# QData/ChromeGCN

Measured on AMD Instinct MI355X. Metric: GCN windows/sec (2-layer, d_model=128) on GM12878 Hi-C graph, higher is better.
Workload: dtype f32

## Files before the change

### chromegcn_amd/csrc/cgcn_head.hip

```cpp
#include "cgcn_common.hpp"

#define HEAD_STAT_BLOCKS 128
#define HEAD_TILE 16
#define HEADB_TILE 32
#ifndef HEAD_MAX_PARTIALS
#define HEAD_MAX_PARTIALS 256
#endif


template <int D>
__global__ __launch_bounds__(256) void k_head_colstats(int n, int S, int rows_per_blk, const float* __restrict__ X,
                                                       float* __restrict__ part) {
  constexpr int RL = 256 / D;
  __shared__ float sm[2][256];
  const int c = threadIdx.x % D, rl = threadIdx.x / D;
  const int r0 = blockIdx.x * rows_per_blk, r1 = min(n, r0 + rows_per_blk);
  for (int s = 0; s < S; ++s) {
    const float* Xs = X + (size_t)s * n * D + c;
    const float pivot = r0 < n ? fmaxf(Xs[(size_t)r0 * D], 0.f) : 0.f;
    float s1 = 0.f, s2 = 0.f;
    int i = r0 + rl;
    for (; i + 3 * RL < r1; i += 4 * RL) {
      float v[4];
#pragma unroll
// ... 1130 lines not shown
#pragma unroll
      for (int t = 0; t < RPW; ++t) {
        const int i = node0 + own + t * 8;
#pragma unroll
        for (int s = 0; s < 2; ++s) {
          if (i < n && s < S) ld_row<EPL>(xv[t][s], &X[(unsigned)((s * n + i) * D + lane * EPL)]);
          else zero_row<EPL>(xv[t][s]);
        }
      }
    };
    auto load_targets = [&](int tile) {
      const int node0 = tile * TR;
      const int j = own * 16 + (lane & 15), q = lane >> 4;
#pragma unroll
      for (int mb = 0; mb < NRB; ++mb)
#pragma unroll
        for (int e = 0; e < 4; ++e) {
          const int i = node0 + mb * 16 + q * 4 + e;
          tgv[mb][e] = (i < n && j < Cp) ? target[(unsigned)(i * C + c0 + j)] : 0.f;
        }
    };
    if (mt > 0) {
      load_rows(blockIdx.x);
      load_targets(blockIdx.x);
    }
    __syncthreads();
#pragma unroll
    for (int e = 0; e < EPL; ++e)
#pragma unroll
      for (int s = 0; s < 2; ++s) head_stat<D>(sa, stash, mean, invstd, s < S ? s : 0, lane * EPL + e, mu[s][e], is[s][e]);
    for (int k = 0; k <= mt; ++k) {
      const int tile = (int)blockIdx.x + k * G;
      const int node0 = tile * TR;
      RS_STAMP(0);
      if (k < mt) {
        int lane_ = lane;
        asm volatile("" : "+v"(lane_));
        float* __restrict__ Yb = Yt[k & 1];
#pragma unroll
        for (int t = 0; t < RPW; ++t) {
          const int rr = own + t * 8;
          const int i = node0 + rr;
          f32x2 ym;
#pragma unroll
          for (int e = 0; e < EPL; ++e) {
            float y[2];
#pragma unroll
            for (int s = 0; s < 2; ++s) {
              y[s] = (fmaxf(xv[t][s][e], 0.f) - mu[s][e]) * is[s][e] * gw[e] + gb[e];
              if (DROP) y[s] = dropout_keep(key, (uint32_t)((s * n + i) * D + lane_ * EPL + e), thresh) ? y[s] * keep_scale : 0.f;
            }
            const float a = y[0] + (S2 ? y[1] : 0.f);
            ym[e] = i < n ? a * invS : 0.f;
          }
          *(f32x2*)&Yb[rr * LDY + lane_ * EPL] = ym;
        }
      }
      RS_STAMP(1);
      __syncthreads();
      RS_STAMP(2);
      f32x4 acc[NRB];
#pragma unroll
      for (int mb = 0; mb < NRB; ++mb) acc[mb] = (f32x4){0.f, 0.f, 0.f, 0.f};
      if (k < mt) {
        if (k + 1 < mt) load_rows(tile + G);
        if (own < NB) {
          OPAQUE_LANE(r, q, lq);
          __builtin_amdgcn_s_setprio(HEAD_RS_PRIO);
          const float* __restrict__ Ya = Yt[k & 1] + r * LDY + 4 * q;
          const float* __restrict__ Wa = Wl + (own * 16 + r) * LDW + 4 * q;
#pragma unroll
          for (int t = 0; t < KQ / 4; ++t) {
            f32x4 a[NRB];
#pragma unroll
            for (int mb = 0; mb < NRB; ++mb) a[mb] = *(const f32x4*)&Ya[mb * 16 * LDY + 16 * t];
            const f32x4 b = *(const f32x4*)&Wa[16 * t];
#pragma unroll
            for (int u = 0; u < 4; ++u)
#pragma unroll
              for (int mb = 0; mb < NRB; ++mb) acc[mb] = __builtin_amdgcn_mfma_f32_16x16x4f32(a[mb][u], b[u], acc[mb], 0, 0, 0);
          }
          __builtin_amdgcn_s_setprio(0);
        }
      }
      RS_STAMP(3);
      __syncthreads();
      RS_STAMP(4);
      if (k < mt) {
        float* __restrict__ Pb = Pt[k & 1];
        OPAQUE_LANE(r, q, lq);
        const int j = own * 16 + r;
#pragma unroll
        for (int mb = 0; mb < NRB; ++mb)
#pragma unroll
          for (int e = 0; e < 4; ++e) {
            const int row = mb * 16 + q * 4 + e;
            const int i = node0 + row;
            const bool ok = i < n && j < Cp;
            const float pred = acc[mb][e] + bj;
            const float en = __expf(-fabsf(pred));
            const float inv = __builtin_amdgcn_rcpf(1.f + en);
            const float p = pred >= 0.f ? inv : en * inv;
            const float l = fmaxf(pred, 0.f) - pred * tgv[mb][e] + __logf(1.f + en);
            lacc += ok ? l : 0.f;
            if (ok) {
              if (HEAD_NT_PROBS) __builtin_nontemporal_store(p, &probs[(unsigned)(i * C + c0 + j)]);
              else probs[(unsigned)(i * C + c0 + j)] = p;
            }
            const float dp = ok ? (p - tgv[mb][e]) * inv_count : 0.f;
            dbo += dp;
            Pb[row * LDP + j] = dp;
          }
        if (k + 1 < mt) load_targets(tile + G);
      }
      RS_STAMP(5);
      __syncthreads();
    }
    dbo += __shfl_xor(dbo, 16);
    dbo += __shfl_xor(dbo, 32);
    if ((lane >> 4) == 0 && c0 + own * 16 + (lane & 15) < CPT) P[CPT * D + c0 + own * 16 + (lane & 15)] = dbo;
    lacc = wave_sum(lacc);
    if (lane == 0) lsum[own] = lacc;
    __syncthreads();
    if (threadIdx.x == 0) {
      float t = 0.f;
#pragma unroll
      for (int w = 0; w < 8; ++w) t += lsum[w];
      const float tl = first ? t : loss_part[blockIdx.x] + t;
      loss_part[blockIdx.x] = tl;
#ifndef HRSX_NOTICKET
      if (sa.acc && last) head_loss_ticket(sa, S, D, tl, inv_count);
#endif
    }
  } else {
    f32x4 accW[NB];
#pragma unroll
    for (int i = 0; i < NB; ++i) accW[i] = (f32x4){0.f, 0.f, 0.f, 0.f};
    float sdy[2] = {0.f, 0.f}, sdyx[2] = {0.f, 0.f}, mu[2], is[2];
    __syncthreads();
    if (sa.acc && blockIdx.x == 0 && first && wave == 8) head_stat_bookkeeping<D>(sa, stash, S, lane);
#pragma unroll
    for (int s = 0; s < 2; ++s) head_stat<D>(sa, stash, mean, invstd, s < S ? s : 0, own * 16 + (lane & 15), mu[s], is[s]);
    float xq[2][NRB][4];
    auto load_xq = [&](int tile) {
      OPAQUE_LANE(r, q, lq);
      const int node0 = tile * TR, c = own * 16 + r;
#pragma unroll
      for (int s = 0; s < 2; ++s)
#pragma unroll
        for (int mb = 0; mb < NRB; ++mb)
#pragma unroll
          for (int e = 0; e < 4; ++e) {
            const int i = node0 + mb * 16 + q * 4 + e;
            xq[s][mb][e] = (last && i < n && s < S) ? X[(unsigned)((s * n + i) * D + c)] : 0.f;
          }
    };
    for (int k = 0; k <= mt; ++k) {
      const int node0 = ((int)blockIdx.x + (k - 1) * G) * TR;
      f32x4 accY[NRB];
#pragma unroll
      for (int mb = 0; mb < NRB; ++mb) accY[mb] = (f32x4){0.f, 0.f, 0.f, 0.f};
      RS_STAMP(0);
      if (k >= 1) {
        const float* __restrict__ Pb = Pt[(k - 1) & 1];
        OPAQUE_LANE(r, q, lq);
        if (MULTI && !first) {
          const int c = own * 16 + r;
#pragma unroll
          for (int mb = 0; mb < NRB; ++mb)
#pragma unroll
            for (int e = 0; e < 4; ++e) {
              const int i = node0 + mb * 16 + q * 4 + e;
              accY[mb][e] = i < n ? dym[(unsigned)(i * D + c)] : 0.f;
            }
        }
        __builtin_amdgcn_s_setprio(HEAD_RS_PRIO);
        const float* __restrict__ Pa = Pb + r * LDP + q;
        const float* __restrict__ Wa = Wl + q * LDW + own * 16 + r;
        float pa[2][4 * NRB], wb[2][4];
#pragma unroll
        for (int u = 0; u < 4; ++u) {
          wb[0][u] = Wa[4 * u * LDW];
#pragma unroll
          for (int mb = 0; mb < NRB; ++mb) pa[0][u * NRB + mb] = Pa[mb * 16 * LDP + 4 * u];
        }
#pragma unroll
        for (int g = 0; g < NB; ++g) {
          if (g + 1 < NB) {
#pragma unroll
            for (int u = 0; u < 4; ++u) {
              wb[(g + 1) & 1][u] = Wa[4 * (4 * (g + 1) + u) * LDW];
#pragma unroll
              for (int mb = 0; mb < NRB; ++mb) pa[(g + 1) & 1][u * NRB + mb] = Pa[mb * 16 * LDP + 4 * (4 * (g + 1) + u)];
            }
          }
          __builtin_amdgcn_sched_barrier(0);
#pragma unroll
          for (int u = 0; u < 4; ++u)
#pragma unroll
            for (int mb = 0; mb < NRB; ++mb) accY[mb] = __builtin_amdgcn_mfma_f32_16x16x4f32(pa[g & 1][u * NRB + mb], wb[g & 1][u], accY[mb], 0, 0, 0);
          __builtin_amdgcn_sched_barrier(0);
        }
        __builtin_amdgcn_s_setprio(0);
      }
      RS_STAMP(1);
      __syncthreads();
      RS_STAMP(2);
      if (k >= 1) {
        OPAQUE_LANE(r, q, lq);
        const int c = own * 16 + r;
#pragma unroll
        for (int mb = 0; mb < NRB; ++mb)
#pragma unroll
          for (int e = 0; e < 4; ++e) {
            const int i = node0 + mb * 16 + q * 4 + e;
            const float g = accY[mb][e];
            if (i < n) dym[(unsigned)(i * D + c)] = g;
            if (last) {
#pragma unroll
              for (int s = 0; s < 2; ++s) {
                float dy = g * invS;
                if (DROP) dy = dropout_keep(key, (uint32_t)((s * n + i) * D + c), thresh) ? dy * keep_scale : 0.f;
                if (s == 1) dy = S2 ? dy : 0.f;
                const float xh = (fmaxf(xq[s][mb][e], 0.f) - mu[s]) * is[s];
                sdy[s] += dy;
                sdyx[s] += dy * xh;
              }
            }
          }
      }
      RS_STAMP(3);
      __syncthreads();
      RS_STAMP(4);
      if (k < mt) load_xq((int)blockIdx.x + k * G);
      if (k >= 1) {
        OPAQUE_LANE(r, q, lq);
        __builtin_amdgcn_s_setprio(HEAD_RS_PRIO);
        const float* __restrict__ Pa = Pt[(k - 1) & 1] + q * LDP + r;
        const float* __restrict__ Ya = Yt[(k - 1) & 1] + q * LDY + own * 16 + r;
        float a0[NB], a1[NB], b0, b1;
        b0 = Ya[0];
#pragma unroll
        for (int ib = 0; ib < NB; ++ib) a0[ib] = Pa[ib * 16];
#pragma unroll
        for (int kk = 0; kk < TR / 4; kk += 2) {
          b1 = Ya[(kk + 1) * 4 * LDY];
#pragma unroll
          for (int ib = 0; ib < NB; ++ib) a1[ib] = Pa[(kk + 1) * 4 * LDP + ib * 16];
          __builtin_amdgcn_sched_barrier(0);
#pragma unroll
          for (int ib = 0; ib < NB; ++ib) accW[ib] = __builtin_amdgcn_mfma_f32_16x16x4f32(a0[ib], b0, accW[ib], 0, 0, 0);
          __builtin_amdgcn_sched_barrier(0);
          if (kk + 2 < TR / 4) {
            b0 = Ya[(kk + 2) * 4 * LDY];
#pragma unroll
            for (int ib = 0; ib < NB; ++ib) a0[ib] = Pa[(kk + 2) * 4 * LDP + ib * 16];
          }
          __builtin_amdgcn_sched_barrier(0);
#pragma unroll
          for (int ib = 0; ib < NB; ++ib) accW[ib] = __builtin_amdgcn_mfma_f32_16x16x4f32(a1[ib], b1, accW[ib], 0, 0, 0);
          __builtin_amdgcn_sched_barrier(0);
        }
        __builtin_amdgcn_s_setprio(0);
      }
      RS_STAMP(5);
      __syncthreads();
    }
    const int r = lane & 15, q = lane >> 4;
#pragma unroll
    for (int ib = 0; ib < CBMAX; ++ib)
#pragma unroll
      for (int e = 0; e < 4; ++e) {
        const float v = ib < NB ? accW[ib < NB ? ib : 0][e] : 0.f;
        if (c0 + ib * 16 < CPT) P[(size_t)(c0 + ib * 16 + q * 4 + e) * D + own * 16 + r] = v;
      }
    if (last) {
      double* out = (double*)(P + CPT * D + CPT);
#pragma unroll
      for (int s = 0; s < 2; ++s) {
        double a = (double)sdy[s], b = (double)sdyx[s];
        a += __shfl_xor(a, 16); a += __shfl_xor(a, 32);
        b += __shfl_xor(b, 16); b += __shfl_xor(b, 32);
        if (q == 0) {
          out[s * D + own * 16 + r] = a;
          out[(2 + s) * D + own * 16 + r] = b;
          if (sa.acc && s < S) {
            int fa, fb;
            head_bacc_points(wmax, 16, keep_scale, n, fa, fb);
            unsigned long long* bb = bacc_base(sa.acc, S, D);
#ifndef HRSX_NOBACC
            bacc_add(bb, S, D, (int)blockIdx.x & (STAT_ACC_SLOTS - 1), s, own * 16 + r, a, b, fa, fb);
#endif
            if (blockIdx.x == 0 && s == 0 && own == 0 && r == 0)
              bb[(size_t)STAT_ACC_SLOTS * S * D * 2 + BACC_EXP] = ((unsigned long long)(unsigned)(fb + 1024) << 32) | (unsigned long long)(unsigned)(fa + 1024);
          }
        }
      }
    }
    __syncthreads();
  }
#undef OPAQUE_LANE
}

#ifndef HEADSP_BARRIERS
#define HEADSP_BARRIERS 2
#endif
template <bool MULTI, int NB, bool DROP>
__global__ __launch_bounds__(1024) void k_head_fused_sp(int n, int S, int C, const float* __restrict__ X,
                                                        const float* __restrict__ bn_w, const float* __restrict__ bn_b,
                                                        const float* __restrict__ mean, const float* __restrict__ invstd,
                                                        const float* __restrict__ Wout, const float* __restrict__ bout,
                                                        const float* __restrict__ target, float keep_scale, uint32_t thresh,
                                                        const unsigned long long* __restrict__ rng_state, float inv_count,
                                                        float* __restrict__ probs, float* __restrict__ loss_part,
                                                        float* __restrict__ dym, float* __restrict__ part,
                                                        int c0, int Cp, int CPT, int first_, int last_, HeadStatAcc sa) {
  constexpr int D = 128, TR = 16, EPL = 2, RPW = TR / 8;
  constexpr int LVT = TR * 256;
  constexpr int WLV = 128 * 256;
  __shared__ __attribute__((aligned(16))) unsigned char Wl[3 * WLV];
  __shared__ __attribute__((aligned(16))) unsigned char Ytb[2][3 * LVT];
  __shared__ __attribute__((aligned(16))) unsigned char Ptb[2][3 * LVT];
  __shared__ float lsum[8];
  __shared__ float wmax[16];
  const bool first = MULTI ? first_ != 0 : true, last = MULTI ? last_ != 0 : true;

  const int lane = threadIdx.x & 63;
  const int wave = __builtin_amdgcn_readfirstlane(threadIdx.x >> 6);
  const int own = wave & 7;
  const uint32_t key = DROP ? dropout_key(rng_state, HEAD_STREAM_ID) : 0u;
  const float invS = 1.f / (float)S;
  const bool S2 = S > 1;
  const int PS = head_part_stride(CPT, D);
  const int ntiles = (n + TR - 1) / TR;
  const int G = (int)gridDim.x;
  const int mt = (int)blockIdx.x < ntiles ? (ntiles - 1 - (int)blockIdx.x) / G + 1 : 0;
  float* P = part + (size_t)blockIdx.x * PS;

  float mwl = 0.f;
  for (int idx = threadIdx.x; idx < 128 * (D / 4); idx += 1024) {
    const int j = idx / (D / 4), c4 = idx % (D / 4);
    f32x4 v = (f32x4){0.f, 0.f, 0.f, 0.f};
    if (j < Cp) v = *(const f32x4*)&Wout[(size_t)(c0 + j) * D + c4 * 4];
    u32x2 h2, m2, l2;
    sp_split4(v, h2, m2, l2);
    unsigned char* w = Wl + j * 256 + (((c4 >> 1) ^ sp_sigma(j & 15)) << 4) + ((c4 & 1) << 3);
    *(u32x2*)w = h2;
    *(u32x2*)(w + WLV) = m2;
    *(u32x2*)(w + 2 * WLV) = l2;
    mwl = fmaxf(fmaxf(mwl, fmaxf(fabsf(v[0]), fabsf(v[1]))), fmaxf(fabsf(v[2]), fabsf(v[3])));
  }
  if (sa.acc && last) {
    float mw;
    if (MULTI) mw = head_wout_absmax(Wout, C * (D / 4), 1024);
    else {
      mw = mwl;
#pragma unroll
      for (int o = 32; o > 0; o >>= 1) mw = fmaxf(mw, __shfl_xor(mw, o, WAVE));
    }
    if ((threadIdx.x & 63) == 0) wmax[threadIdx.x >> 6] = mw;
  }
  float* const stash = (float*)Ptb[1];
  static_assert(3 * LVT >= 6 * D * (int)sizeof(float), "the stash fits a P tile");
#ifndef HRSX_NOSTAGE
  if (sa.acc) head_stat_stage<D>(sa, n, S, stash, 1024);
#endif
#define OPAQUE_LANE(r_, q_, l_)          \
  int l_ = lane;                         \
  asm volatile("" : "+v"(l_));           \
  const int r_ = l_ & 15, q_ = l_ >> 4

  if (wave < 8) {
    float xv[RPW][2][EPL], tgv[4], mu[2][EPL], is[2][EPL], gw[EPL], gb[EPL];
    float dbo = 0.f, lacc = 0.f;
    const float bj = own * 16 + (lane & 15) < Cp ? bout[c0 + own * 16 + (lane & 15)] : 0.f;
#pragma unroll
    for (int e = 0; e < EPL; ++e) {
      const int c = lane * EPL + e;
      gw[e] = bn_w[c];
      gb[e] = bn_b[c];
    }
    bf16x8 wh[4], wm[4], wl[4];
    {
      const int r = lane & 15, q = lane >> 4;
      const int j = own * 16 + r;
#pragma unroll
      for (int s4 = 0; s4 < 4; ++s4) {
        f32x4 v0 = {0.f, 0.f, 0.f, 0.f}, v1 = v0;
        if (j < Cp) {
          v0 = *(const f32x4*)&Wout[(size_t)(c0 + j) * D + 32 * s4 + 8 * q];
          v1 = *(const f32x4*)&Wout[(size_t)(c0 + j) * D + 32 * s4 + 8 * q + 4];
        }
        const float v[8] = {v0[0], v0[1], v0[2], v0[3], v1[0], v1[1], v1[2], v1[3]};
        sp_split8(v, wh[s4], wm[s4], wl[s4]);
      }
    }
    auto load_rows = [&](int tile) {
      const int node0 = tile * TR;
#pragma unroll
      for (int t = 0; t < RPW; ++t) {
        const int i = node0 + own + t * 8;
#pragma unroll
        for (int s = 0; s < 2; ++s) {
          if (i < n && s < S) ld_row<EPL>(xv[t][s], &X[(unsigned)((s * n + i) * D + lane * EPL)]);
          else zero_row<EPL>(xv[t][s]);
        }
      }
    };
    auto load_targets = [&](int tile) {
      const int node0 = tile * TR;
      const int j = own * 16 + (lane & 15), q = lane >> 4;
#pragma unroll
      for (int e = 0; e < 4; ++e) {
        const int i = node0 + q * 4 + e;
        tgv[e] = (i < n && j < Cp) ? target[(unsigned)(i * C + c0 + j)] : 0.f;
      }
    };
    if (mt > 0) {
      load_rows(blockIdx.x);
      load_targets(blockIdx.x);
    }
    __syncthreads();
#pragma unroll
    for (int e = 0; e < EPL; ++e)
#pragma unroll
      for (int s = 0; s < 2; ++s) head_stat<D>(sa, stash, mean, invstd, s < S ? s : 0, lane * EPL + e, mu[s][e], is[s][e]);
    for (int k = 0; k <= mt; ++k) {
      const int tile = (int)blockIdx.x + k * G;
      const int node0 = tile * TR;
      if (k < mt) {
        int lane_ = lane;
        asm volatile("" : "+v"(lane_));
        unsigned char* __restrict__ Yb = Ytb[k & 1];
#pragma unroll
        for (int t = 0; t < RPW; ++t) {
          const int rr = own + t * 8;
          const int i = node0 + rr;
          float ym[EPL];
#pragma unroll
          for (int e = 0; e < EPL; ++e) {
            float y[2];
#pragma unroll
            for (int s = 0; s < 2; ++s) {
              y[s] = (fmaxf(xv[t][s][e], 0.f) - mu[s][e]) * is[s][e] * gw[e] + gb[e];
              if (DROP) y[s] = dropout_keep(key, (uint32_t)((s * n + i) * D + lane_ * EPL + e), thresh) ? y[s] * keep_scale : 0.f;
            }
            const float a = y[0] + (S2 ? y[1] : 0.f);
            ym[e] = i < n ? a * invS : 0.f;
          }
          uint32_t yh, ymid, yl;
          sp_split2(ym[0], ym[1], yh, ymid, yl);
          unsigned char* w = Yb + rr * 256 + (((lane_ >> 2) ^ sp_sigma(rr)) << 4) + ((lane_ & 3) << 2);
          *(uint32_t*)w = yh;
          *(uint32_t*)(w + LVT) = ymid;
          *(uint32_t*)(w + 2 * LVT) = yl;
        }
      }
      __syncthreads();
      f32x4 acc = {0.f, 0.f, 0.f, 0.f};
      if (k < mt) {
        if (k + 1 < mt) load_rows(tile + G);
        if (own < NB) {
          OPAQUE_LANE(r, q, lq);
          const unsigned char* __restrict__ Ya = Ytb[k & 1] + r * 256 + ((q ^ (sp_sigma(r) & 3)) << 4);
          const int hi = sp_sigma(r) >> 2;
          SpAcc sacc;
          sacc.zero();
#pragma unroll
          for (int s4 = 0; s4 < 4; ++s4) {
            const int o = (s4 ^ hi) << 6;
            const bf16x8 ah = __builtin_bit_cast(bf16x8, *(const u32x4*)(Ya + o));
            const bf16x8 am = __builtin_bit_cast(bf16x8, *(const u32x4*)(Ya + LVT + o));
            const bf16x8 al = __builtin_bit_cast(bf16x8, *(const u32x4*)(Ya + 2 * LVT + o));
            sacc.step(ah, am, al, wh[s4], wm[s4], wl[s4]);
          }
          acc = sacc.sum();
        }
      }
#if HEADSP_BARRIERS == 3
      __syncthreads();
#endif
      if (k < mt) {
        unsigned char* __restrict__ Pb = Ptb[k & 1];
        OPAQUE_LANE(r, q, lq);
        const int j = own * 16 + r;
#pragma unroll
        for (int e = 0; e < 4; ++e) {
          const int row = q * 4 + e;
          const int i = node0 + row;
          const bool ok = i < n && j < Cp;
          const float pred = acc[e] + bj;
          const float en = __expf(-fabsf(pred));
          const float inv = __builtin_amdgcn_rcpf(1.f + en);
          const float p = pred >= 0.f ? inv : en * inv;
          const float l = fmaxf(pred, 0.f) - pred * tgv[e] + __logf(1.f + en);
          lacc += ok ? l : 0.f;
          if (ok) {
            if (HEAD_NT_PROBS) __builtin_nontemporal_store(p, &probs[(unsigned)(i * C + c0 + j)]);
            else probs[(unsigned)(i * C + c0 + j)] = p;
          }
          const float dp = ok ? (p - tgv[e]) * inv_count : 0.f;
          dbo += dp;
          uint16_t dh, dm, dl;
          sp_split1(dp, dh, dm, dl);
          unsigned char* w = Pb + row * 256 + (((j >> 3) ^ sp_sigma(row)) << 4) + ((j & 7) << 1);
          *(uint16_t*)w = dh;
          *(uint16_t*)(w + LVT) = dm;
          *(uint16_t*)(w + 2 * LVT) = dl;
        }
        if (k + 1 < mt) load_targets(tile + G);
      }
      __syncthreads();
    }
    dbo += __shfl_xor(dbo, 16);
    dbo += __shfl_xor(dbo, 32);
    if ((lane >> 4) == 0 && c0 + own * 16 + (lane & 15) < CPT) P[CPT * D + c0 + own * 16 + (lane & 15)] = dbo;
    lacc = wave_sum(lacc);
    if (lane == 0) lsum[own] = lacc;
    __syncthreads();
    if (threadIdx.x == 0) {
      float t = 0.f;
#pragma unroll
      for (int w = 0; w < 8; ++w) t += lsum[w];
      const float tl = first ? t : loss_part[blockIdx.x] + t;
      loss_part[blockIdx.x] = tl;
#ifndef HRSX_NOTICKET
      if (sa.acc && last) head_loss_ticket(sa, S, D, tl, inv_count);
#endif
    }
  } else {
    f32x16 accW[2];
#pragma unroll
    for (int bb = 0; bb < 2; ++bb)
#pragma unroll
      for (int e = 0; e < 16; ++e) accW[bb][e] = 0.f;
    float sdy[2] = {0.f, 0.f}, sdyx[2] = {0.f, 0.f}, mu[2], is[2];
    __syncthreads();
    if (sa.acc && blockIdx.x == 0 && first && wave == 8) head_stat_bookkeeping<D>(sa, stash, S, lane);
#pragma unroll
    for (int s = 0; s < 2; ++s) head_stat<D>(sa, stash, mean, invstd, s < S ? s : 0, own * 16 + (lane & 15), mu[s], is[s]);
    float xq[2][4];
    auto load_xq = [&](int tile) {
      OPAQUE_LANE(r, q, lq);
      const int node0 = tile * TR, c = own * 16 + r;
#pragma unroll
      for (int s = 0; s < 2; ++s)
#pragma unroll
        for (int e = 0; e < 4; ++e) {
          const int i = node0 + q * 4 + e;
          xq[s][e] = (last && i < n && s < S) ? X[(unsigned)((s * n + i) * D + c)] : 0.f;
        }
    };
    for (int k = 0; k <= mt; ++k) {
      const int node0 = ((int)blockIdx.x + (k - 1) * G) * TR;
      f32x4 accY = {0.f, 0.f, 0.f, 0.f};
      if (k >= 1) {
        const unsigned char* __restrict__ Pb = Ptb[(k - 1) & 1];
        OPAQUE_LANE(r, q, lq);
        const unsigned char* __restrict__ Pa = Pb + r * 256 + ((q ^ (sp_sigma(r) & 3)) << 4);
        const int hi = sp_sigma(r) >> 2;
        const int qp = r >> 2, pp = r & 3;
        SpAcc2 sacc;
        sacc.zero();
#pragma unroll
        for (int s4 = 0; s4 < 4; ++s4) {
          const int o = (s4 ^ hi) << 6;
          const bf16x8 ah = __builtin_bit_cast(bf16x8, *(const u32x4*)(Pa + o));
          const bf16x8 am = __builtin_bit_cast(bf16x8, *(const u32x4*)(Pa + LVT + o));
          const bf16x8 al = __builtin_bit_cast(bf16x8, *(const u32x4*)(Pa + 2 * LVT + o));
          int wo[2];
#pragma unroll
          for (int rd = 0; rd < 2; ++rd) {
            const int lrow = 32 * s4 + 8 * q + 4 * rd + qp;
            wo[rd] = lrow * 256 + (((2 * own + (pp >> 1)) ^ sp_sigma(lrow & 15)) << 4) + ((pp & 1) << 3);
          }
          const bf16x8 bh = tr_pair(Wl + wo[0], Wl + wo[1]);
          const bf16x8 bm = tr_pair(Wl + WLV + wo[0], Wl + WLV + wo[1]);
          const bf16x8 bl = tr_pair(Wl + 2 * WLV + wo[0], Wl + 2 * WLV + wo[1]);
          sacc.step(ah, am, al, bh, bm, bl);
        }
        accY = sacc.sum();
        if (MULTI && !first) {
          const int c = own * 16 + r;
#pragma unroll
          for (int e = 0; e < 4; ++e) {
            const int i = node0 + q * 4 + e;
            accY[e] += i < n ? dym[(unsigned)(i * D + c)] : 0.f;
          }
        }
      }
#if HEADSP_BARRIERS == 3
      __syncthreads();
#endif
      if (k >= 1) {
        OPAQUE_LANE(r, q, lq);
        const int c = own * 16 + r;
#pragma unroll
        for (int e = 0; e < 4; ++e) {
          const int i = node0 + q * 4 + e;
          const float g = accY[e];
          if (i < n) dym[(unsigned)(i * D + c)] = g;
          if (last) {
#pragma unroll
            for (int s = 0; s < 2; ++s) {
              float dy = g * invS;
              if (DROP) dy = dropout_keep(key, (uint32_t)((s * n + i) * D + c), thresh) ? dy * keep_scale : 0.f;
              if (s == 1) dy = S2 ? dy : 0.f;
              const float xh = (fmaxf(xq[s][e], 0.f) - mu[s]) * is[s];
              sdy[s] += dy;
              sdyx[s] += dy * xh;
            }
          }
        }
      }
      __syncthreads();
      if (k < mt) load_xq((int)blockIdx.x + k * G);
      if (k >= 1) {
        int lq = lane;
        asm volatile("" : "+v"(lq));
        const int hh = lq >> 5, c16 = (lq >> 4) & 1, qp = (lq & 15) >> 2, pp = lq & 3;
        const int cbk = own >> 1, lb0 = 2 * (own & 1);
        const unsigned char* __restrict__ Pb = Ptb[(k - 1) & 1];
        const unsigned char* __restrict__ Yb = Ytb[(k - 1) & 1];
        int ty[2], tp[2];
#pragma unroll
        for (int rd = 0; rd < 2; ++rd) {
          const int row = 8 * hh + 4 * rd + qp, sg = sp_sigma(row);
          ty[rd] = row * 256 + (((4 * cbk + 2 * c16 + (pp >> 1)) ^ sg) << 4) + ((pp & 1) << 3);
          tp[rd] = row * 256 + (((4 * lb0 + 2 * c16 + (pp >> 1)) ^ sg) << 4) + ((pp & 1) << 3);
        }
        bf16x8 yf[3];
#pragma unroll
        for (int v = 0; v < 3; ++v) yf[v] = tr_pair(Yb + v * LVT + ty[0], Yb + v * LVT + ty[1]);
#pragma unroll
        for (int bb = 0; bb < 2; ++bb) {
          bf16x8 pf[3];
#pragma unroll
          for (int v = 0; v < 3; ++v) pf[v] = tr_pair(Pb + v * LVT + (tp[0] ^ (bb << 6)), Pb + v * LVT + (tp[1] ^ (bb << 6)));
          accW[bb] = __builtin_amdgcn_mfma_f32_32x32x16_bf16(pf[2], yf[0], accW[bb], 0, 0, 0);
          accW[bb] = __builtin_amdgcn_mfma_f32_32x32x16_bf16(pf[0], yf[2], accW[bb], 0, 0, 0);
          accW[bb] = __builtin_amdgcn_mfma_f32_32x32x16_bf16(pf[1], yf[1], accW[bb], 0, 0, 0);
          accW[bb] = __builtin_amdgcn_mfma_f32_32x32x16_bf16(pf[1], yf[0], accW[bb], 0, 0, 0);
          accW[bb] = __builtin_amdgcn_mfma_f32_32x32x16_bf16(pf[0], yf[1], accW[bb], 0, 0, 0);
          accW[bb] = __builtin_amdgcn_mfma_f32_32x32x16_bf16(pf[0], yf[0], accW[bb], 0, 0, 0);
        }
      }
      __syncthreads();
    }
    {
      const int hh = lane >> 5, cbk = own >> 1, lb0 = 2 * (own & 1);
#pragma unroll
      for (int bb = 0; bb < 2; ++bb)
#pragma unroll
        for (int e = 0; e < 16; ++e) {
          const int lab = 32 * (lb0 + bb) + (e & 3) + 8 * (e >> 2) + 4 * hh;
          if (c0 + (lab & ~15) < CPT) P[(size_t)(c0 + lab) * D + 32 * cbk + (lane & 31)] = accW[bb][e];
        }
    }
    const int r = lane & 15, q = lane >> 4;
    if (last) {
      double* out = (double*)(P + CPT * D + CPT);
#pragma unroll
      for (int s = 0; s < 2; ++s) {
        double a = (double)sdy[s], b = (double)sdyx[s];
        a += __shfl_xor(a, 16); a += __shfl_xor(a, 32);
        b += __shfl_xor(b, 16); b += __shfl_xor(b, 32);
        if (q == 0) {
          out[s * D + own * 16 + r] = a;
          out[(2 + s) * D + own * 16 + r] = b;
          if (sa.acc && s < S) {
            int fa, fb;
            head_bacc_points(wmax, 16, keep_scale, n, fa, fb);
            unsigned long long* bb = bacc_base(sa.acc, S, D);
#ifndef HRSX_NOBACC
            bacc_add(bb, S, D, (int)blockIdx.x & (STAT_ACC_SLOTS - 1), s, own * 16 + r, a, b, fa, fb);
#endif
            if (blockIdx.x == 0 && s == 0 && own == 0 && r == 0)
              bb[(size_t)STAT_ACC_SLOTS * S * D * 2 + BACC_EXP] = ((unsigned long long)(unsigned)(fb + 1024) << 32) | (unsigned long long)(unsigned)(fa + 1024);
          }
        }
      }
    }
    __syncthreads();
  }
#undef OPAQUE_LANE
}

__global__ __launch_bounds__(512) void k_head_bwd_finalize(int wslab0, int wslabs, int P, int n, int S, int D, int C, int CP,
                                                           const float* __restrict__ part, float* __restrict__ dWout,
                                                           float* __restrict__ dbout, float* __restrict__ dbn_w,
                                                           float* __restrict__ dbn_b, float* __restrict__ bnc,
                                                           int accumulate, const float* __restrict__ dloss) {
  if ((int)blockIdx.x < wslabs)
    head_finalize_slab<512>(wslab0 + blockIdx.x, P, D, C, CP, part, dWout, dbout, accumulate, dloss);
  else
    head_stats_finalize<512>((int)blockIdx.x - wslabs, P, n, S, D, CP, part, dbn_w, dbn_b, bnc, accumulate, dloss);
}

__global__ __launch_bounds__(512) void k_head_train_finish(int P, int n, int S, int D, int CP,
                                                           const float* __restrict__ part, float* __restrict__ bnc,
                                                           const float* __restrict__ loss_part, float inv_count,
                                                           float* __restrict__ loss) {
  if (blockIdx.x == 0) {
    __shared__ float sm[512];
    float s = 0.f;
    for (int i = threadIdx.x; i < P; i += 512) s += loss_part[i];
    sm[threadIdx.x] = s;
    __syncthreads();
    for (int o = 256; o > 0; o >>= 1) {
      if ((int)threadIdx.x < o) sm[threadIdx.x] += sm[threadIdx.x + o];
      __syncthreads();
    }
    if (threadIdx.x == 0) loss[0] = sm[0] * inv_count;
    return;
  }
  head_stats_finalize<512>((int)blockIdx.x - 1, P, n, S, D, CP, part, nullptr, nullptr, bnc, 0, nullptr);
}

template <int D>
__global__ __launch_bounds__(256) void k_head_bn_bwd_apply(int n, int S, const float* __restrict__ X,
                                                           const float* __restrict__ bn_w, const float* __restrict__ mean,
                                                           const float* __restrict__ invstd, const float* __restrict__ dym,
                                                           const float* __restrict__ bnc, float keep_scale, uint32_t thresh,
                                                           const unsigned long long* __restrict__ rng_state,
                                                           float* __restrict__ dX) {
  const uint32_t key = thresh ? dropout_key(rng_state, HEAD_STREAM_ID) : 0u;
  const size_t total4 = (size_t)S * n * D / 4;
  const float invS = 1.f / (float)S;
  for (size_t v = (size_t)blockIdx.x * blockDim.x + threadIdx.x; v < total4; v += (size_t)gridDim.x * blockDim.x) {
    const size_t el0 = v * 4;
    const int c0 = (int)(el0 % D);
    const size_t row = el0 / D;
    const int s = (int)(row / n);
    const int i = (int)(row % n);
    const f32x4 x = *(const f32x4*)&X[el0];
    const f32x4 g = *(const f32x4*)&dym[(size_t)i * D + c0];
    f32x4 o;
#pragma unroll
    for (int e = 0; e < 4; ++e) {
      const int c = c0 + e;
      float dy = g[e] * invS;
      if (thresh) dy = dropout_keep(key, (uint32_t)(el0 + e), thresh) ? dy * keep_scale : 0.f;
      const float is = invstd[s * D + c];
      const float xh = (fmaxf(x[e], 0.f) - mean[s * D + c]) * is;
      const float dr = bn_w[c] * is * (dy - bnc[(s * 2 + 0) * D + c] - xh * bnc[(s * 2 + 1) * D + c]);
      o[e] = x[e] > 0.f ? dr : 0.f;
    }
    *(f32x4*)&dX[el0] = o;
  }
}

static int head_check(int n, int S, int d, int C) {
  if (n < 0 || C < 1) return CGCN_ERR_BAD_ARG;
  if (!(S == 1 || S == 2) || !(d == 128 || d == 256) || C > 256) return CGCN_ERR_UNSUPPORTED;
  if ((double)n * S * d * 4.0 >= 4294967296.0 || (double)n * C * 4.0 >= 4294967296.0) return CGCN_ERR_UNSUPPORTED;
  return CGCN_OK;
}
static inline int head_cp(int C) { return C <= 128 ? 128 : 256; }
static inline int head_stat_blocks(int n, int* rows_per_blk) {
  int rpb = (n + HEAD_STAT_BLOCKS - 1) / HEAD_STAT_BLOCKS;
  if (rpb < 8) rpb = 8;
  *rows_per_blk = rpb;
  int nb = (n + rpb - 1) / rpb;
  return nb < 1 ? 1 : nb;
}
static inline int head_bwd_partials(int n) {
  int t = (n + HEADB_TILE - 1) / HEADB_TILE;
  if (t > HEAD_MAX_PARTIALS) t = HEAD_MAX_PARTIALS;
  return t < 1 ? 1 : t;
}
static inline size_t ws_stats(int S, int d) { return (size_t)HEAD_STAT_BLOCKS * S * d * 2; }
static inline size_t ws_loss(int n) { return (size_t)((n + HEAD_TILE - 1) / HEAD_TILE + 4); }
static inline size_t ws_dym(int n, int d) { return (size_t)n * d + 4; }
static inline size_t ws_bnc(int d) { return (size_t)2 * 2 * d; }
static inline size_t ws_part(int n, int d, int C) { return (size_t)head_bwd_partials(n) * (size_t)head_part_stride(head_cp(C), d); }
static inline size_t align4(size_t x) { return (x + 3) & ~(size_t)3; }

extern "C" {

#ifdef HF_TIMING
int cgcn_debug_hf_stamps(unsigned long long* out) {
  return hipMemcpyFromSymbol(out, HIP_SYMBOL(hf_stamps), sizeof(unsigned long long) * 8 * 16) == hipSuccess ? 0 : -1;
}
#endif


int cgcn_head_workspace_layout(int n, int S, int d, int C, size_t* dym_offset, size_t* bnc_offset, size_t* part_offset) {
  int rc = head_check(n, S, d, C);
  if (rc) return rc;
  if (!dym_offset || !bnc_offset || !part_offset) return CGCN_ERR_BAD_ARG;
  *dym_offset = 4 * (align4(ws_stats(S, d)) + align4(ws_loss(n)));
  *bnc_offset = *dym_offset + 4 * align4(ws_dym(n, d));
  *part_offset = *bnc_offset + 4 * align4(ws_bnc(d));
  return CGCN_OK;
}

int cgcn_head_bwd_partials(int n) { return head_bwd_partials(n); }

size_t cgcn_head_workspace_bytes(int n, int S, int d, int C) {
  if (head_check(n, S, d, C) != CGCN_OK) return 0;
  return 4 * (align4(ws_stats(S, d)) + align4(ws_loss(n)) + align4(ws_dym(n, d)) + align4(ws_bnc(d)) + align4(ws_part(n, d, C)));
}

int cgcn_head_fwd(cgcn_stream_t stream, int n, int S, int d, int C, const float* X, const float* bn_w,
                  const float* bn_b, float* run_mean, float* run_var, long long* num_batches_tracked, float momentum,
                  float eps, int training, const float* Wout, const float* bout, const float* target, float dropout_p,
                  const unsigned long long* rng_state, float* probs, float* loss, float* dpred, float* save_mean,
                  float* save_invstd, void* workspace, size_t workspace_bytes) {
  int rc = head_check(n, S, d, C);
  if (rc) return rc;
  if (!X || !bn_w || !bn_b || !Wout || !bout || !target || !probs || !loss || !workspace) return CGCN_ERR_BAD_ARG;
  if (!run_mean || !run_var) return CGCN_ERR_BAD_ARG;
  if (training && (!save_mean || !save_invstd || n < 2)) return CGCN_ERR_BAD_ARG;
  const bool drop = training && dropout_p > 0.f;
  if (drop && (!rng_state || dropout_p >= 1.f)) return CGCN_ERR_BAD_ARG;
  if (workspace_bytes < cgcn_head_workspace_bytes(n, S, d, C)) return CGCN_ERR_WORKSPACE;
  if (misaligned16(Wout) || misaligned16(workspace) || misaligned16(X)) return CGCN_ERR_BAD_ARG;
  hipStream_t st = (hipStream_t)stream;
  float* w_stats = (float*)workspace;
  float* w_loss = w_stats + align4(ws_stats(S, d));
  if (n == 0) {
    hipLaunchKernelGGL(k_sum_scale, dim3(1), dim3(256), 0, st, 0, w_loss, 0.f, loss);
    return launch_status();
  }
  if (training) {
    int rpb;
    const int nblk = head_stat_blocks(n, &rpb);
    if (d == 128) hipLaunchKernelGGL((k_head_colstats<128>), dim3(nblk), dim3(256), 0, st, n, S, rpb, X, w_stats);
    else hipLaunchKernelGGL((k_head_colstats<256>), dim3(nblk), dim3(256), 0, st, n, S, rpb, X, w_stats);
    if ((rc = launch_status())) return rc;
    launch_bn_finalize(st, n, S, d, nblk, rpb, w_stats, momentum, eps, run_mean, run_var, num_batches_tracked, save_mean, save_invstd);
    if ((rc = launch_status())) return rc;
  }
  const int blocks = (n + HEAD_TILE - 1) / HEAD_TILE;
  const float keep_scale = drop ? 1.f / (1.f - dropout_p) : 1.f;
  const uint32_t thresh = drop ? dropout_threshold(dropout_p) : 0u;
  const float inv_count = 1.f / ((float)n * (float)C);
  const float* mean = training ? save_mean : run_mean;
  const float* vr = training ? save_invstd : run_var;
#define HF(D_, NC_)                                                                                                   \
  hipLaunchKernelGGL((k_head_fwd<D_, NC_>), dim3(blocks), dim3(512), 0, st, n, S, C, X, bn_w, bn_b, mean, vr,         \
                     training ? 0 : 1, eps, Wout, bout, target, keep_scale, thresh, rng_state, inv_count, probs,      \
                     training ? dpred : nullptr, w_loss, nullptr)
  if (d == 128) { if (C <= 128) HF(128, 1); else HF(128, 2); }
  else { if (C <= 128) HF(256, 1); else HF(256, 2); }
#undef HF
  if ((rc = launch_status())) return rc;
  hipLaunchKernelGGL(k_sum_scale, dim3(1), dim3(256), 0, st, blocks, w_loss, inv_count, loss);
  return launch_status();
}

int cgcn_head_logits(cgcn_stream_t stream, int n, int S, int d, int C, const float* X, const float* bn_w,
                     const float* bn_b, const float* run_mean, const float* run_var, float eps, const float* Wout,
                     const float* bout, float* logits) {
  int rc = head_check(n, S, d, C);
  if (rc) return rc;
  if (!X || !bn_w || !bn_b || !run_mean || !run_var || !Wout || !bout || !logits) return CGCN_ERR_BAD_ARG;
  if (misaligned16(Wout) || misaligned16(X)) return CGCN_ERR_BAD_ARG;
  if (n == 0) return CGCN_OK;
  hipStream_t st = (hipStream_t)stream;
  const int blocks = (n + HEAD_TILE - 1) / HEAD_TILE;
  for (int s = 0; s < S; ++s) {
    const float* Xs = X + (size_t)s * n * d;
    float* Ls = logits + (size_t)s * n * C;
#define HF(D_, NC_)                                                                                                   \
  hipLaunchKernelGGL((k_head_fwd<D_, NC_>), dim3(blocks), dim3(512), 0, st, n, 1, C, Xs, bn_w, bn_b, run_mean, run_var, \
                     1, eps, Wout, bout, nullptr, 1.f, 0u, nullptr, 0.f, nullptr, nullptr, nullptr, Ls)
    if (d == 128) { if (C <= 128) HF(128, 1); else HF(128, 2); }
    else { if (C <= 128) HF(256, 1); else HF(256, 2); }
#undef HF
    if ((rc = launch_status())) return rc;
  }
  return CGCN_OK;
}

}

static int head_train_impl(cgcn_stream_t stream, int n, int S, int d, int C, const float* X, const float* bn_w,
                    const float* bn_b, float* run_mean, float* run_var, long long* num_batches_tracked, float momentum,
                    float eps, const float* Wout, const float* bout, const float* target, float dropout_p,
                    const unsigned long long* rng_state, float* probs, float* loss, float* save_mean, float* save_invstd,
                    const float* col_stats, int col_stats_tiles, int col_stats_rows, void* workspace,
                    size_t workspace_bytes, int phases) {
  int rc = head_check(n, S, d, C);
  if (rc) return rc;
  if (!X || !bn_w || !bn_b || !Wout || !bout || !target || !probs || !loss || !workspace || !run_mean || !run_var ||
      !save_mean || !save_invstd || n < 2)
    return CGCN_ERR_BAD_ARG;
  const size_t acc_tile_bytes = (size_t)S * d * 2 * sizeof(float);
  const bool stat_acc = col_stats && col_stats_rows == -1;
  if (stat_acc && ((size_t)col_stats_tiles * acc_tile_bytes < stat_acc_words(S, d) * 8 || ((uintptr_t)col_stats & 7)))
    return CGCN_ERR_BAD_ARG;
  if (col_stats && !stat_acc && (col_stats_rows < 1 || col_stats_tiles != (n + col_stats_rows - 1) / col_stats_rows)) return CGCN_ERR_BAD_ARG;
  const bool drop = dropout_p > 0.f;
  if (drop && (!rng_state || dropout_p >= 1.f)) return CGCN_ERR_BAD_ARG;
  if (workspace_bytes < cgcn_head_workspace_bytes(n, S, d, C)) return CGCN_ERR_WORKSPACE;
// ... 165 lines not shown
```

Before: 62.77 million.

## Keep split Wout fragments in registers for backward waves, drop Wl LDS buffer

Removes the 96KB shared-memory Wl staging of the three-way bf16-split output weights. The backward waves now load and split their transposed Wout fragments straight into registers once, instead of doing transposed LDS reads for every tile. The weight abs-max is now computed during each wave's register load. This cuts LDS traffic and footprint, which could allow more blocks per CU, but it adds register pressure and strided uncoalesced global loads of Wout at kernel start. It also drops the optional third-barrier variant.

Result: no change. 63.28 million (median of 6 runs) (+0.8%).

```diff
diff --git a/chromegcn_amd/csrc/cgcn_head.hip b/chromegcn_amd/csrc/cgcn_head.hip
--- a/chromegcn_amd/csrc/cgcn_head.hip
+++ b/chromegcn_amd/csrc/cgcn_head.hip
@@ -1456,9 +1456,6 @@
 #undef OPAQUE_LANE
 }
 
-#ifndef HEADSP_BARRIERS
-#define HEADSP_BARRIERS 2
-#endif
 template <bool MULTI, int NB, bool DROP>
 __global__ __launch_bounds__(1024) void k_head_fused_sp(int n, int S, int C, const float* __restrict__ X,
                                                         const float* __restrict__ bn_w, const float* __restrict__ bn_b,
@@ -1471,8 +1468,6 @@
                                                         int c0, int Cp, int CPT, int first_, int last_, HeadStatAcc sa) {
   constexpr int D = 128, TR = 16, EPL = 2, RPW = TR / 8;
   constexpr int LVT = TR * 256;
-  constexpr int WLV = 128 * 256;
-  __shared__ __attribute__((aligned(16))) unsigned char Wl[3 * WLV];
   __shared__ __attribute__((aligned(16))) unsigned char Ytb[2][3 * LVT];
   __shared__ __attribute__((aligned(16))) unsigned char Ptb[2][3 * LVT];
   __shared__ float lsum[8];
@@ -1491,29 +1486,22 @@
   const int mt = (int)blockIdx.x < ntiles ? (ntiles - 1 - (int)blockIdx.x) / G + 1 : 0;
   float* P = part + (size_t)blockIdx.x * PS;
 
-  float mwl = 0.f;
-  for (int idx = threadIdx.x; idx < 128 * (D / 4); idx += 1024) {
-    const int j = idx / (D / 4), c4 = idx % (D / 4);
-    f32x4 v = (f32x4){0.f, 0.f, 0.f, 0.f};
-    if (j < Cp) v = *(const f32x4*)&Wout[(size_t)(c0 + j) * D + c4 * 4];
-    u32x2 h2, m2, l2;
-    sp_split4(v, h2, m2, l2);
-    unsigned char* w = Wl + j * 256 + (((c4 >> 1) ^ sp_sigma(j & 15)) << 4) + ((c4 & 1) << 3);
-    *(u32x2*)w = h2;
-    *(u32x2*)(w + WLV) = m2;
-    *(u32x2*)(w + 2 * WLV) = l2;
-    mwl = fmaxf(fmaxf(mwl, fmaxf(fabsf(v[0]), fabsf(v[1]))), fmaxf(fabsf(v[2]), fabsf(v[3])));
-  }
-  if (sa.acc && last) {
-    float mw;
-    if (MULTI) mw = head_wout_absmax(Wout, C * (D / 4), 1024);
-    else {
-      mw = mwl;
+  const bool want_wmax = sa.acc && last;
+  if (MULTI && want_wmax) {
+    const float mw = head_wout_absmax(Wout, C * (D / 4), 1024);
+    if ((threadIdx.x & 63) == 0) wmax[threadIdx.x >> 6] = mw;
+  }
+  auto put_wmax = [&](const float (&v)[8], float& mw) {
+#pragma unroll
+    for (int u = 0; u < 8; ++u) mw = fmaxf(mw, fabsf(v[u]));
+  };
+  auto merge_wmax = [&](float mw) {
+    if (!MULTI && want_wmax) {
 #pragma unroll
       for (int o = 32; o > 0; o >>= 1) mw = fmaxf(mw, __shfl_xor(mw, o, WAVE));
-    }
-    if ((threadIdx.x & 63) == 0) wmax[threadIdx.x >> 6] = mw;
-  }
+      if (lane == 0) wmax[wave] = mw;
+    }
+  };
   float* const stash = (float*)Ptb[1];
   static_assert(3 * LVT >= 6 * D * (int)sizeof(float), "the stash fits a P tile");
 #ifndef HRSX_NOSTAGE
@@ -1538,6 +1526,7 @@
     {
       const int r = lane & 15, q = lane >> 4;
       const int j = own * 16 + r;
+      float mw = 0.f;
 #pragma unroll
       for (int s4 = 0; s4 < 4; ++s4) {
         f32x4 v0 = {0.f, 0.f, 0.f, 0.f}, v1 = v0;
@@ -1547,7 +1536,9 @@
         }
         const float v[8] = {v0[0], v0[1], v0[2], v0[3], v1[0], v1[1], v1[2], v1[3]};
         sp_split8(v, wh[s4], wm[s4], wl[s4]);
-      }
+        put_wmax(v, mw);
+      }
+      merge_wmax(mw);
     }
     auto load_rows = [&](int tile) {
       const int node0 = tile * TR;
@@ -1631,9 +1622,6 @@
           acc = sacc.sum();
         }
       }
-#if HEADSP_BARRIERS == 3
-      __syncthreads();
-#endif
       if (k < mt) {
         unsigned char* __restrict__ Pb = Ptb[k & 1];
         OPAQUE_LANE(r, q, lq);
@@ -1689,6 +1677,24 @@
 #pragma unroll
       for (int e = 0; e < 16; ++e) accW[bb][e] = 0.f;
     float sdy[2] = {0.f, 0.f}, sdyx[2] = {0.f, 0.f}, mu[2], is[2];
+    bf16x8 bh[4], bm[4], bl[4];
+    {
+      const int r = lane & 15, q = lane >> 4;
+      float mw = 0.f;
+#pragma unroll
+      for (int s4 = 0; s4 < 4; ++s4) {
+        float v[8];
+#pragma unroll
+        for (int u = 0; u < 8; ++u) {
+          const int j = 32 * s4 + 8 * q + u;
+          const float w = Wout[(size_t)(c0 + (j < Cp ? j : Cp - 1)) * D + own * 16 + r];
+          v[u] = j < Cp ? w : 0.f;
+        }
+        sp_split8(v, bh[s4], bm[s4], bl[s4]);
+        put_wmax(v, mw);
+      }
+      merge_wmax(mw);
+    }
     __syncthreads();
     if (sa.acc && blockIdx.x == 0 && first && wave == 8) head_stat_bookkeeping<D>(sa, stash, S, lane);
 #pragma unroll
@@ -1713,7 +1719,6 @@
         OPAQUE_LANE(r, q, lq);
         const unsigned char* __restrict__ Pa = Pb + r * 256 + ((q ^ (sp_sigma(r) & 3)) << 4);
         const int hi = sp_sigma(r) >> 2;
-        const int qp = r >> 2, pp = r & 3;
         SpAcc2 sacc;
         sacc.zero();
 #pragma unroll
@@ -1722,16 +1727,7 @@
           const bf16x8 ah = __builtin_bit_cast(bf16x8, *(const u32x4*)(Pa + o));
           const bf16x8 am = __builtin_bit_cast(bf16x8, *(const u32x4*)(Pa + LVT + o));
           const bf16x8 al = __builtin_bit_cast(bf16x8, *(const u32x4*)(Pa + 2 * LVT + o));
-          int wo[2];
-#pragma unroll
-          for (int rd = 0; rd < 2; ++rd) {
-            const int lrow = 32 * s4 + 8 * q + 4 * rd + qp;
-            wo[rd] = lrow * 256 + (((2 * own + (pp >> 1)) ^ sp_sigma(lrow & 15)) << 4) + ((pp & 1) << 3);
-          }
-          const bf16x8 bh = tr_pair(Wl + wo[0], Wl + wo[1]);
-          const bf16x8 bm = tr_pair(Wl + WLV + wo[0], Wl + WLV + wo[1]);
-          const bf16x8 bl = tr_pair(Wl + 2 * WLV + wo[0], Wl + 2 * WLV + wo[1]);
-          sacc.step(ah, am, al, bh, bm, bl);
+          sacc.step(ah, am, al, bh[s4], bm[s4], bl[s4]);
         }
         accY = sacc.sum();
         if (MULTI && !first) {
@@ -1743,9 +1739,6 @@
           }
         }
       }
-#if HEADSP_BARRIERS == 3
-      __syncthreads();
-#endif
       if (k >= 1) {
         OPAQUE_LANE(r, q, lq);
         const int c = own * 16 + r;
```
